# GuoleiSun/VSS-CFFM

Hardware: AMD Instinct MI355X
Metric: clips/sec (fwd+bwd) CFFM-B1 480x480 T=4 hot path (CFFA+CFM, decoder_focal depth 2) (higher is better)
Workload: dtype f32 in/out, f32 accumulate; MFMA operands: split-bf16 (hi+lo, ~2^-17) in the Linear GEMMs, f16 in QK^T/AV

## Files before the change

vss_cffm_amd/csrc/cffm_hip.hip:

```cpp
#include "cfm_attn_kernels.h"
#include "clip_kernels.h"
#include "rowops_kernels.h"
#include "gtc_kernels.h"
#include "gemm.h"
#include "segfuse_kernels.h"
#include "segloss_kernels.h"
#include "headfuse_kernels.h"
#include "kmeans_kernels.h"

#include <stdarg.h>
#include <stdio.h>

#include "../../include/cffm_hip.h"

static thread_local char g_err[512] = "";

static int fail(int code, const char* fmt, ...) {
    va_list ap;
    va_start(ap, fmt);
    vsnprintf(g_err, sizeof(g_err), fmt, ap);
    va_end(ap);
    return code;
}
#define CHECK_LAUNCH(name)                                                                        \
// ... 1061 lines not shown
    }
#endif
    CFFM_LAUNCH(k_gtc_attn_bwd, (nwg, CFFM_HEADS, B), (256), (size_t)gtb_lds(K), st, q_raw, q_b, kv_raw, kv_b, o, dout, lse, dq_raw, rec, T, K);
    CFFM_LAUNCH(k_gtc_dkv_sum, (K, CFFM_HEADS, B), (64), 0, st, (const float*)rec, nwg, K, dkv);
    CHECK_LAUNCH("gtc_attn_bwd");
    return 0;
}

#ifndef MLP_MT
#define MLP_MT 2
#endif
#define MLP_D 4
static int mlp_lds_grant() {
#ifndef CFFM_EMU
    static bool granted = false;
    if (!granted) {
        if (hipFuncSetAttribute((const void*)k_mlp_fwd<MLP_MT, MLP_D>, hipFuncAttributeMaxDynamicSharedMemorySize, PNL_FUSED_LDS(MLP_MT)) != hipSuccess ||
            hipFuncSetAttribute((const void*)k_mlp_bwd<MLP_MT, MLP_D>, hipFuncAttributeMaxDynamicSharedMemorySize, PNL_FUSED_LDS(MLP_MT)) != hipSuccess)
            return -1;
        granted = true;
    }
#endif
    return 0;
}
static int panel_mt(long M) {
    const long w2 = (M + 31) / 32, w3 = (M + 47) / 48;
    return ((w3 + 255) / 256) * 3 < ((w2 + 255) / 256) * 2 ? 3 : 2;
}
extern "C++" {
template <int MT, int NTW, bool A_PRE, int EPI>
static int panel_gemm_launch(const float* A, int lda, long M, int K, const float* wf, float* Cout, int ldc, const float* bias, void* aux,
                             hipStream_t st, float* colrec = nullptr, float* a_t = nullptr) {
    auto kern = k_panel_gemm<MT, NTW, 2, 4, A_PRE, EPI>;
#ifndef CFFM_EMU
    static bool granted = false;
    if (!granted) {
        if (hipFuncSetAttribute((const void*)kern, hipFuncAttributeMaxDynamicSharedMemorySize, PNL_LDS(MT)) != hipSuccess) return -1;
        granted = true;
    }
#endif
    CFFM_LAUNCH(kern, ((unsigned)((M + 16 * MT - 1) / (16 * MT))), (PNL_THREADS), PNL_LDS(MT), st, A, lda, (int)M, K, (const f32x4*)wf, Cout, ldc, bias, aux, colrec, (f32x4*)a_t);
    return 0;
}
}
static int panel_qkv_fwd(const float* x_s, const float* wf, const float* b, h16* qkv16, long M, hipStream_t st, float* x_t = nullptr) {
    return panel_mt(M) == 3 ? panel_gemm_launch<3, 6, true, 3>(x_s, 256, M, 256, wf, nullptr, 768, b, qkv16, st, nullptr, x_t)
                            : panel_gemm_launch<2, 6, true, 3>(x_s, 256, M, 256, wf, nullptr, 768, b, qkv16, st, nullptr, x_t);
}
static long panel_qkv_records(long M) { return (M + 16 * panel_mt(M) - 1) / (16 * panel_mt(M)); }
static int panel_qkv_dx(const float* dqkv, const float* wfn, float* dx, long M, hipStream_t st, float* colrec = nullptr, float* dqkv_t = nullptr) {
    return panel_mt(M) == 3 ? panel_gemm_launch<3, 2, false, 0>(dqkv, 768, M, 768, wfn, dx, 256, nullptr, nullptr, st, colrec, dqkv_t)
                            : panel_gemm_launch<2, 2, false, 0>(dqkv, 768, M, 768, wfn, dx, 256, nullptr, nullptr, st, colrec, dqkv_t);
}
#ifndef CFFM_DW_STREAM_DEFAULT
#define CFFM_DW_STREAM_DEFAULT 0
#endif
static int g_dw_stream = CFFM_DW_STREAM_DEFAULT;
static int dw_stream_sw() { return g_dw_stream; }
int cffm_dw_stream(int on) { const int was = g_dw_stream; if (on >= 0) g_dw_stream = on != 0; return was; }

static long cffm_mlp_records(long NP) { return (NP + 16 * MLP_MT - 1) / (16 * MLP_MT); }

int cffm_panel_pack_weight(const float* w, int N, int K, int form, float* w_frag, void* stream) {
    REQUIRE(w && w_frag && N >= 16 && K >= 16 && N % 32 == 0 && K % 32 == 0 && (form == 0 || form == 1), "panel_pack_weight: bad arguments");
    CFFM_LAUNCH(k_pnl_pack_weight, ((unsigned)(((long)N * K / 8 + 255) / 256)), (256), 0, (hipStream_t)stream, w, N, K, form, (f32x4*)w_frag);
    CHECK_LAUNCH("panel_pack_weight");
    return 0;
}

static int cffm_mlp_fwd_tfrag(const float* ao, const float* xt, long xt_bs, int rows_per_batch, const float* wp_f, const float* w1_f, const float* w2_f,
                              const float* bp, const float* b1, const float* b2, const float* g2, const float* be2, float* x1, float* z2s, float* mean2,
                              float* rstd2, float* hraw, float* acts, float* x2, float* ao_t, float* z2_t, float* act_t, long NP, void* stream) {
    REQUIRE(NP >= 0 && NP < (1L << 21) && rows_per_batch >= 1, "mlp_fwd: bad sizes");
    if (!NP) return 0;
    REQUIRE(ao && xt && wp_f && w1_f && w2_f && bp && b1 && b2 && g2 && be2 && x1 && mean2 && rstd2 && hraw && x2, "mlp_fwd: null");
    REQUIRE(!mlp_lds_grant(), "mlp_fwd: LDS grant failed");
    PROF2(ST_MLP_FWD);
    MlpFwdArgs a;
    a.ao = ao; a.xt = xt; a.xt_bs = xt_bs; a.rows_per_batch = rows_per_batch;
    a.wp = (const f32x4*)wp_f; a.w1 = (const f32x4*)w1_f; a.w2 = (const f32x4*)w2_f;
    a.bp = bp; a.b1 = b1; a.b2 = b2; a.g2 = g2; a.be2 = be2;
    a.x1 = x1; a.z2s = z2s; a.mean2 = mean2; a.rstd2 = rstd2; a.hraw = hraw; a.acts = acts; a.x2 = x2; a.NP = (int)NP;
    a.ao_t = (f32x4*)ao_t; a.z2_t = (f32x4*)z2_t; a.act_t = (f32x4*)act_t;
    CFFM_LAUNCH((k_mlp_fwd<MLP_MT, MLP_D>), ((unsigned)cffm_mlp_records(NP)), (PNL_THREADS), PNL_FUSED_LDS(MLP_MT), (hipStream_t)stream, a);
    CHECK_LAUNCH("mlp_fwd");
    return 0;
}
int cffm_mlp_fwd(const float* ao, const float* xt, long xt_bs, int rows_per_batch, const float* wp_f, const float* w1_f, const float* w2_f,
                 const float* bp, const float* b1, const float* b2, const float* g2, const float* be2, float* x1, float* z2s, float* mean2,
                 float* rstd2, float* hraw, float* acts, float* x2, long NP, void* stream) {
    REQUIRE(z2s || !NP, "mlp_fwd: null");
    return cffm_mlp_fwd_tfrag(ao, xt, xt_bs, rows_per_batch, wp_f, w1_f, w2_f, bp, b1, b2, g2, be2, x1, z2s, mean2, rstd2, hraw, acts, x2, nullptr, nullptr,
                              nullptr, NP, stream);
}

static int cffm_mlp_bwd_tfrag(const float* dout, const float* hraw, const float* b1, const float* x1, const float* mean2, const float* rstd2,
                              const float* g2, const float* w2_n, const float* w1_n, const float* wp_n, float* dhs, float* dx1, float* dao, float* dg2,
                              float* dbe2, float* db1, float* db2, float* dbp, float* dout_t, float* dh_t, float* dx1_t, long NP, void* stream) {
    REQUIRE(NP >= 0 && NP < (1L << 21), "mlp_bwd: bad sizes");
    if (!NP) return 0;
    REQUIRE(dout && hraw && b1 && x1 && mean2 && rstd2 && g2 && w2_n && w1_n && wp_n && dx1 && dao, "mlp_bwd: null");
    REQUIRE(!mlp_lds_grant(), "mlp_bwd: LDS grant failed");
    PROF2(ST_MLP_BWD);
    hipStream_t st = (hipStream_t)stream;
    const int nrec = (int)cffm_mlp_records(NP);
    float* rec = red_scratch((size_t)nrec * 2048, st);
// ... 327 lines not shown
        DwsPlan P4;
        if (stream_dw && dw_stream_plan(all4, 4, dw_stream_target(), &P4)) need = P4.part_floats;
        REQUIRE(!need || lib_scratch2(need), "block_backward: scratch allocation failed");
    }
    auto dw_group = [&](const cffm_wgrad* wg, const GemmTNPre* pre, int n, hipStream_t s, int target, void (*after)(hipStream_t)) -> int {
        if (!stream_dw) return gemm_tn_group((const GemmTN*)wg, n, s, pre, s == st ? lib_scratch : lib_scratch2, target, after);
        DwsPlan P;
        if (!dw_stream_plan((const GemmTN*)wg, n, dw_stream_target(), &P)) return -1;
        float* part = P.part_floats ? (s == st ? lib_scratch : lib_scratch2)(P.part_floats) : nullptr;
        if (P.part_floats && !part) return -1;
        return dw_group_stream((const GemmTN*)wg, n, s, part, dw_stream_target(), after);
    };
    const cffm_wgrad wg_qkv = {stream_dw ? dqkv_t : dqkv, stream_dw ? ws + L.zall_t : ws + L.zall, gr->qkv_w, NR, 768, CFFM_C};
    const cffm_wgrad wg_fc1 = {dact, ws + L.z2, gr->fc1_w, NP, CFFM_HID, CFFM_C};
    const cffm_wgrad wg_fc2 = {stream_dw ? dout_t : dout, ws + L.act, gr->fc2_w, NP, CFFM_C, CFFM_HID};
    const cffm_wgrad wg_proj = {stream_dw ? dx1_t : dx1, stream_dw ? ws + L.ao_t : ws + L.ao, gr->proj_w, NP, CFFM_C, CFFM_C};
    {
        const float* wfn = ws + L.w_frag + PREP_WFLOATS;
        PROF(ST_GEMM);
        if (stream_dw)
            TRY(cffm_mlp_bwd_tfrag(dout, ws + L.hraw, p->fc1_b, ws + L.x1, ws + L.mean2, ws + L.rstd2, p->norm2_w, wfn + 768 * 256 + 256 * 256 + 1024 * 256,
                                   wfn + 768 * 256 + 256 * 256, wfn + 768 * 256, nullptr, dx1, dao, gr->norm2_w, gr->norm2_b, gr->fc1_b, gr->fc2_b, gr->proj_b,
                                   dout_t, dact, dx1_t, NP, stream));
        else
        TRY(cffm_mlp_bwd(dout, ws + L.hraw, p->fc1_b, ws + L.x1, ws + L.mean2, ws + L.rstd2, p->norm2_w, wfn + 768 * 256 + 256 * 256 + 1024 * 256,
                         wfn + 768 * 256 + 256 * 256, wfn + 768 * 256, dact, dx1, dao, gr->norm2_w, gr->norm2_b, gr->fc1_b, gr->fc2_b, gr->proj_b, NP,
                         stream));
        TRY(tail_flush(st));
        if (!one_group) {
            sa = side_fork(st, 0);
            void* stream_a = (void*)sa;
            const cffm_wgrad wga[2] = {wg_fc1, wg_fc2};
            const GemmTNPre prea[2] = {{1, 1, nullptr}, {0, 1, p->fc1_b}};
            {
                void* stream = stream_a;
                PROF2(ST_G_DW);
                REQUIRE(!dw_group(wga, prea, 2, sa, 320, nullptr), "block_backward: weight-gradient gemm failed");
            }
            side_mark(sa, st, 0);
        }
    }
    hipStream_t sb = st, s1 = st;
    float* dbp;
    int ng;
    {
        PROF(ST_ATTN_BWD);
#ifndef CFFM_EMU
        if (g_side.bias_pending[par]) {
            side_wait(st, g_side.bias_done[par]);
            g_side.bias_pending[par] = false;
        }
#endif
        TRY(attn_bwd_fused(g, ws + L.qkv, key_src, q_dst, (const h16*)(ws + L.bias), ws + L.ao, dao, ws + L.lse, dqkv, scratch + S.dkvp, &dbp, &ng, par, stream));
        TRY(attn_bwd_gather(g, inv_ptr, inv_idx, scratch + S.dkvp, dqkv, stream));
    }
    const long nrec = panel_qkv_records(NR);
    float* qkv_rec = red_scratch((size_t)nrec * 768, st);
    REQUIRE(qkv_rec, "block_backward: scratch allocation failed");
    {
        RedSegs segs;
        segs.nseg = 0;
        seg_add(segs, 0, 768, gr->qkv_b, 0);
        reduce_records(qkv_rec, (int)nrec, 768, 768, segs, st);
    }
    {
        if (!stream_dw) side_fork_mark(st, 2);
        PROF(ST_GEMM); PROF2(ST_G_QKV_DX);
        REQUIRE(!panel_qkv_dx(dqkv, ws + L.w_frag + PREP_WFLOATS, dzall, NR, st, qkv_rec, stream_dw ? dqkv_t : nullptr), "block_backward: q|k|v input-gradient gemm failed");
        if (stream_dw) side_fork_mark(st, 2);
    }
    auto side_b = [&]() -> int {
        sb = side_fork_take(st, 2);
        void* stream_b = (void*)sb;
        if (one_group) {
            const cffm_wgrad wg4[4] = {wg_qkv, wg_fc1, wg_fc2, wg_proj};
            const GemmTNPre pre4[4] = {{0, 1, nullptr}, {1, 1, nullptr}, {0, 1, p->fc1_b}, {0, 0, nullptr}};
            void* stream = stream_b;
            PROF(ST_GEMM); PROF2(ST_G_DW);
            REQUIRE(!dw_group(wg4, pre4, 4, sb, 480, dw_group_launched), "block_backward: weight-gradient gemm failed");
            sa = sb;
            side_mark(sa, st, 0);
            {
                PROF(ST_ATTN_BWD);
                s1 = sb;
                TRY(attn_bwd_bias_sum(dbp, ng, dbiasT, (void*)s1));
                TRY(cffm_bias_scatter(dbiasT, gr->rpb_own, gr->rpb_ring, gr->rpb_pool, (void*)s1));
            }
        } else {
            const cffm_wgrad wgb[2] = {wg_qkv, wg_proj};
            const GemmTNPre preb[2] = {{0, 1, nullptr}, {0, 0, nullptr}};
            {
                void* stream = stream_b;
                PROF(ST_GEMM); PROF2(ST_G_DW);
                REQUIRE(!dw_group(wgb, preb, 2, sb, 320, dw_group_launched), "block_backward: weight-gradient gemm failed");
            }
            PROF(ST_ATTN_BWD);
            s1 = sb;
            TRY(attn_bwd_bias_sum(dbp, ng, dbiasT, (void*)s1));
            TRY(cffm_bias_scatter(dbiasT, gr->rpb_own, gr->rpb_ring, gr->rpb_pool, (void*)s1));
        }
        return 0;
    };
    const bool side_late = stream_dw && one_group;
    if (!side_late) TRY(side_b());
    if (!side_late && (!one_group || dx_tgt == dout)) side_join(sa, st, 0);
#ifndef CFFM_EMU
    if (g_side.dw_pending[par ^ 1] && g_side.dw_dout[par ^ 1] == dx_tgt) {
        side_wait(st, g_side.dw_done[par ^ 1]);
        g_side.dw_pending[par ^ 1] = false;
    }
#endif
    TRY(ln_pool_bwd_tgt(g, x_tgt, tgt_bs, p->norm1_w, p->norm1_b, ws + L.M, ws + L.mean1, ws + L.rstd1, dzall, dx1, dx_tgt, dtgt_bs, cffa.rec,
                        stream));
    if (side_late) TRY(side_b());
#ifndef CFFM_EMU
    if (defer && sb != st && s1 != st && g_side.on) {
        if (g_tail.has) TRY(tail_flush(st));
        side_fork_mark(st, 3);
        if (s1 != sb) side_order(s1, sb);
        (void)hipEventRecord(g_side.tail_order, sb);
        g_tail.has = true; g_tail.jobs = g_rq.jobs; g_tail.parity = g_red_parity;
        g_rq.jobs.njob = 0; g_rq.active = false;
        g_side.dw_pending[par] = true;
        g_side.dw_dout[par] = dout;
        side_record(s1, st, g_side.bias_done[par]);
        g_side.bias_pending[par] = true;
        return 0;
    }
#endif
    hipStream_t s3 = side_fork(st, 3);
    if (sb != st && s3 != st) side_order(sb, s3);
    if (s1 != st && s3 != st && s1 != s3) side_order(s1, s3);
    reductions.finish_on(s3);
    CHECK_LAUNCH("block_backward reductions");
#ifndef CFFM_EMU
    if (defer && sb != st && s3 != st) {
        g_side.dw_pending[par] = true;
        g_side.dw_dout[par] = dout;
        side_record(s1, st, g_side.bias_done[par]);
        g_side.bias_pending[par] = s1 != st;
        side_record(s3, st, g_side.tail_done[g_red_parity]);
        g_side.tail_pending[g_red_parity] = true;
        return 0;
    }
#endif
    (void)defer;
    side_mark(s3, st, 1);
    side_join(s3, st, 1);
    if (sb != st && sb != s3) { side_mark(sb, st, 0); side_join(sb, st, 0); }
    return 0;
}

static int segf_maps(SegfMaps& mp, const int* h, const int* w, int nmaps, int H, int W, const char* who) {
    if (nmaps < 0 || nmaps > 3 || H < 1 || W < 1) return fail(-1, "%s: bad map count / size", who);
    mp.cnt = nmaps;
    mp.nseg = 0; mp.per_frame = 0;
// ... 797 lines not shown
```

vss_cffm_amd/csrc/cfm_attn_kernels.h:

```cpp
#pragma once
#include "cffa_kernels.h"

#define ATT_KS_STRIDE 32
#define ATT_SWZ(row) ((0x78 >> (((row) >> 1) & 6)) & 3)
#define ATT_ROW(row, chunk) ((row) * ATT_KS_STRIDE + 8 * ((chunk) ^ ATT_SWZ(row)))

__device__ __forceinline__ f32x4 vflag4(const float* vflag, int o) { return *(const f32x4*)(vflag + o); }
#define CFFM_FIRST_POOLED_KEY 181
#define ATT_FWD_LDS (2 * CFFM_NKEY_PAD * ATT_KS_STRIDE * sizeof(f16) + CFFM_NKEY_PAD * 4)
template <int NROWS = 0>
__device__ __forceinline__ f16x8 att_tr_frag(const f16* img, int r0, int c0, int lane) {
    const int i = lane & 15, row = r0 + 4 * (lane >> 4) + (i >> 2), col = c0 + 4 * (i & 3);
    int row2 = row + 16;
    if (NROWS > 0 && row2 >= NROWS) row2 -= 16;
    const f16x4 a = lds_tr4(img + ATT_ROW(row, col >> 3) + (col & 7));
    const f16x4 b = lds_tr4(img + ATT_ROW(row2, col >> 3) + (col & 7));
    return cat_f16x4(a, b);
}

__device__ __forceinline__ int att_tr_lane(int c0, int lane) {
    const int i = lane & 15, row = 4 * (lane >> 4) + (i >> 2), col = c0 + 4 * (i & 3);
    return ATT_ROW(row, col >> 3) + (col & 7);
}
__device__ __forceinline__ f16x8 att_tr_frag_at(const f16* img_r0, int lane_off, bool clamp_second = false) {
// ... 355 lines not shown
        if (wb == wb0 || ntile == 0) wait_vm0(); else if (ntile == 1) wait_vm<2>(); else wait_vm<4>();
        __syncthreads();
        const bool more = wb + 1 < wb1;
        if (more) dma_rows(n1, onx, bi ^ 1);
        const f16* Ks = img + bi * ATT_BK_IMG;
        const f16* Vs = Ks + CFFM_NKEY_PAD * ATT_KS_STRIDE;
        const f16* Q = Qs + bi * 64 * ATT_KS_STRIDE;
        const f16* dO = dOs + bi * 64 * ATT_KS_STRIDE;
        const float isc = sisc[bi];
#pragma unroll
        for (int u = 0; u < 2; ++u) {
            const int t = t0 + u;
            if (u < ntile) {
                sched_fence();
                const f16x8 kf = *(const f16x8*)(Ks + 512 * t + lrow);
                const f16x8 vf = *(const f16x8*)(Vs + 512 * t + lrow);
                const float mk = t >= 11 ? vfl[bi * CFFM_NKEY_PAD + 16 * t + l15] : 0.f;
                const f32x4 c0 = (f32x4){mk, mk, mk, mk};
                f16x4 ph[4], dsh[4];
#pragma unroll
                for (int qt = 0; qt < 4; ++qt) {
                    if (u == 0 && more) dma_piece(n1.b, onx, bi ^ 1, qt);
                    const f16x8 qf = *(const f16x8*)(Q + 512 * qt + lrow);
                    const f16x8 dof = *(const f16x8*)(dO + 512 * qt + lrow);
                    const f32x4 sv = mfma16x16x32_f16(qf, kf, mfma16x16x32_f16(bT[qt], u ? sel1 : sel0, c0));
                    const f32x4 dp = mfma16x16x32_f16(dof, vf, (f32x4){0.f, 0.f, 0.f, 0.f});
                    const f32x4 lq = *(const f32x4*)(lse2 + bi * 64 + 16 * qt + 4 * g), Dq = *(const f32x4*)(sD + bi * 64 + 16 * qt + 4 * g);
                    f32x4 pr, ds;
#pragma unroll
                    for (int r = 0; r < 4; ++r) {
                        pr[r] = fast_exp2(fmaf(sv[r], CFFM_LOG2E, -lq[r]));
                        ds[r] = pr[r] * (dp[r] - Dq[r]);
                    }
                    dB[u][qt] += ds * isc;
                    ph[qt] = to_f16x4(pr);
                    dsh[qt] = to_f16x4(ds);
                    *(f16x4*)(DS + (qt >> 1) * ATT_BK_DSROWS * ATT_KS_STRIDE + 512 * t + ((qt & 1) ? dsw1 : dsw0)) = dsh[qt];
                }
                if (u == 0 && more) {
                    dma_piece(n1.b, onx, bi ^ 1, 4);
                    if (wb + 3 < wb1) tab_issue(n3.w, r3);
                }
                f32x4 aK[2] = {(f32x4){0.f, 0.f, 0.f, 0.f}, (f32x4){0.f, 0.f, 0.f, 0.f}}, aV[2] = {aK[0], aK[0]};
#pragma unroll
                for (int a = 0; a < 2; ++a) {
                    const f16x8 pf = cat_f16x4(ph[2 * a], ph[2 * a + 1]), dsf = cat_f16x4(dsh[2 * a], dsh[2 * a + 1]);
#pragma unroll
                    for (int mt = 0; mt < 2; ++mt) {
                        aV[mt] = mfma16x16x32_f16(att_tr_frag_at(dO + 1024 * a, mt ? ltp1 : ltp0), pf, aV[mt]);
                        aK[mt] = mfma16x16x32_f16(att_tr_frag_at(Q + 1024 * a, mt ? ltp1 : ltp0), dsf, aK[mt]);
                    }
                }
                const uint32_t so = (uint32_t)(((long)wb * CFFM_NKEY_PAD + 16 * t) * 1024);
                const uint32_t vo = mk == 0.f ? (uint32_t)(l15 * 1024 + (h * 2 * CFFM_HD + 8 * g) * 2) : BUF_OOB;
                buf_st16_pair(rs_part, __builtin_bit_cast(f32x4, cat_f16x4(to_f16x4(aK[0]), to_f16x4(aK[1]))),
                              __builtin_bit_cast(f32x4, cat_f16x4(to_f16x4(aV[0]), to_f16x4(aV[1]))), vo, so, so + 64);
            }
        }
        if (more && ntile == 0) {
#pragma unroll
            for (int k = 0; k < 5; ++k) dma_piece(n1.b, onx, bi ^ 1, k);
            if (wb + 3 < wb1) tab_issue(n3.w, r3);
        }
        if (wb + 2 < wb1) {
            Ahead a;
            sched_fence();
            ahead_lds(r3 + 2 >= 3 ? r3 - 1 : r3 + 2, a);
            dma_prep(n2.w, a, onx);
        }
        if (more && wave < 9) {
            if (wave < 7) wait_vm<8>(); else if (wave == 7) wait_vm<6>(); else wait_vm<4>();
            if (wave < 8) rows_max();
        }
        __syncthreads();
        if (wave >= 8) {
            if (more) rows_convert(wb + 1, bi ^ 1);
        } else {
            const int qt = wave & 3, mt = wave >> 2;
            const f16* D = DS + (qt >> 1) * ATT_BK_DSROWS * ATT_KS_STRIDE;
            const int la = mt ? ltr1 : ltr0, lb = (qt & 1) ? ltr1 : ltr0;
            f32x4 dq = (f32x4){0.f, 0.f, 0.f, 0.f};
#pragma unroll
            for (int p = 0; p < 10; ++p)
                dq = mfma16x16x32_f16(att_tr_frag_at(Ks + 1024 * p, la, p == 9), att_tr_frag_at(D + 1024 * p, lb), dq);
            const int q = 16 * qt + l15;
            if (q < CFFM_WA)
                *(f32x4*)(dqkv + ((long)b * G.RC + w * CFFM_WA + q) * 768 + h * CFFM_HD + 16 * mt + 4 * g) = dq * (scale * isc);
        }
        cur = n1;
        r3 = r3 == 2 ? 0 : r3 + 1;
    }
    const buf_t rs_dbp = buf_make(dbias_part + (((long)grp * CFFM_HEADS + h) * CFFM_NKEY_PAD) * CFFM_NQ_PAD,
                                  (uint32_t)(CFFM_NKEY_PAD * CFFM_NQ_PAD * 4));
#pragma unroll
    for (int u = 0; u < 2; ++u)
#pragma unroll
        for (int qt = 0; qt < 4; qt += 2)
            if (u < ntile) {
                const uint32_t so = (uint32_t)(((16 * (t0 + u)) * CFFM_NQ_PAD + 16 * qt) * 4);
                buf_st16_pair(rs_dbp, dB[u][qt], dB[u][qt + 1], (uint32_t)((l15 * CFFM_NQ_PAD + 4 * g) * 4), so, so + 64);
            }
}

__global__ void __launch_bounds__(256) k_dkv_gather(Geo G, const int* __restrict__ inv_ptr, const int* __restrict__ inv_idx,
                                                     const float* __restrict__ dkv_part, float* __restrict__ dqkv) {
    const int lane = threadIdx.x & 63, row = blockIdx.x * 4 + (threadIdx.x >> 6), b = blockIdx.y;
    if (row >= G.RC) return;
    const int e0 = inv_ptr[row], e1 = inv_ptr[row + 1];
    const h16* part = (const h16*)dkv_part + (long)b * G.nW * CFFM_NKEY_PAD * 512 + 8 * lane;
    const float* scl = dkv_part + (long)G.B * G.nW * CFFM_NKEY_PAD * 256 + (long)b * G.nW * CFFM_HEADS + (lane >> 3);
    f32x4 a0 = (f32x4){0.f, 0.f, 0.f, 0.f}, a1 = a0;
    for (int eb = e0; eb < e1; eb += 64) {
        const int n = (e1 - eb < 64) ? e1 - eb : 64;
        const int mine = (lane < n) ? inv_idx[eb + lane] : 0;
        int e = 0;
        for (; e + 3 < n; e += 4) {
            const int i0 = __shfl(mine, e, 64), i1 = __shfl(mine, e + 1, 64), i2 = __shfl(mine, e + 2, 64), i3 = __shfl(mine, e + 3, 64);
            const h16x8 x0 = *(const h16x8*)(part + (long)i0 * 512), x1 = *(const h16x8*)(part + (long)i1 * 512);
            const h16x8 x2 = *(const h16x8*)(part + (long)i2 * 512), x3 = *(const h16x8*)(part + (long)i3 * 512);
            const float s0 = scl[(i0 / CFFM_NKEY_PAD) * CFFM_HEADS], s1 = scl[(i1 / CFFM_NKEY_PAD) * CFFM_HEADS];
            const float s2 = scl[(i2 / CFFM_NKEY_PAD) * CFFM_HEADS], s3 = scl[(i3 / CFFM_NKEY_PAD) * CFFM_HEADS];
#pragma unroll
            for (int c = 0; c < 4; ++c) {
                a0[c] += ((float)x0[c] * s0 + (float)x1[c] * s1) + ((float)x2[c] * s2 + (float)x3[c] * s3);
                a1[c] += ((float)x0[4 + c] * s0 + (float)x1[4 + c] * s1) + ((float)x2[4 + c] * s2 + (float)x3[4 + c] * s3);
            }
        }
        for (; e < n; ++e) {
            const int i0 = __shfl(mine, e, 64);
            const h16x8 x0 = *(const h16x8*)(part + (long)i0 * 512);
            const float s0 = scl[(i0 / CFFM_NKEY_PAD) * CFFM_HEADS];
#pragma unroll
            for (int c = 0; c < 4; ++c) { a0[c] += (float)x0[c] * s0; a1[c] += (float)x0[4 + c] * s0; }
        }
    }
    float* drow = dqkv + ((long)b * G.RC + row) * 768;
    const int dcol = 256 + 256 * ((lane >> 2) & 1) + CFFM_HD * (lane >> 3) + 8 * (lane & 3);
    *(f32x4*)(drow + dcol) = a0;
    *(f32x4*)(drow + dcol + 4) = a1;
    if (row >= CFFM_WA * G.nW) *(f32x4*)(drow + 4 * lane) = (f32x4){0.f, 0.f, 0.f, 0.f};
}
```

vss_cffm_amd/csrc/panel_kernels.h:

```cpp
#pragma once
#include "cffm_common.h"
#include "gemm_kernels.h"
#include "dws_kernels.h"

#define PNL_KC 256
#define PNL_THREADS 512
#define PNL_WAVES 8
__device__ __forceinline__ int pnl_off(int row, int chunk) { return row * PNL_KC + (((chunk ^ row) & 15) << 3) + ((chunk & 16) << 3); }
#define PNL_IMG(MT) (16 * (MT) * PNL_KC)
#define PNL_LDS(MT) (2 * 2 * PNL_IMG(MT) * 2 + 2 * PNL_THREADS * 16)

__device__ __host__ __forceinline__ long pnl_frag_unit(int jt, int ks, int h, int KS) { return ((long)(jt * KS + ks) * 2 + h) * 64; }

__device__ __forceinline__ void pnl_pack_weight(const float* __restrict__ W, int N, int K, bool nn, f32x4* __restrict__ dst, long item) {
    const int lane = (int)(item & 63);
    const long u = item >> 6;
    const int OUT = nn ? K : N, KS = (nn ? N : K) / 32;
    const int ks = (int)(u % KS), jt = (int)(u / KS);
    if (jt * 16 >= OUT) return;
    const int l15 = lane & 15, g = lane >> 4;
    bf16x8 hi, lo;
#pragma unroll
    for (int e = 0; e < 8; ++e) {
        const int o = 16 * jt + l15, c = 32 * ks + 8 * g + e;
        const float x = nn ? W[(long)c * K + o] : W[(long)o * K + c];
        hi[e] = (bf16)x;
        lo[e] = (bf16)(x - (float)hi[e]);
    }
    dst[pnl_frag_unit(jt, ks, 0, KS) + lane] = __builtin_bit_cast(f32x4, hi);
    dst[pnl_frag_unit(jt, ks, 1, KS) + lane] = __builtin_bit_cast(f32x4, lo);
}
__global__ void __launch_bounds__(256) k_pnl_pack_weight(const float* __restrict__ W, int N, int K, int nn, f32x4* __restrict__ dst) {
    const long item = (long)blockIdx.x * 256 + threadIdx.x;
    if (item < (long)N * K / 8) pnl_pack_weight(W, N, K, nn != 0, dst, item);
}

struct PnlPackJobs { const float* w[4]; f32x4* dst[4]; int N[4], K[4]; long end[4]; int n, nn; };
__global__ void __launch_bounds__(256) k_pnl_pack_weights(PnlPackJobs J) {
    long item = (long)blockIdx.x * 256 + threadIdx.x;
    int j = 0;
#pragma unroll
    for (int q = 0; q < 3; ++q)
        if (q + 1 < J.n && item >= J.end[q]) j = q + 1;
    if (j > 0) item -= J.end[j - 1];
    if (item < (long)J.N[j] * J.K[j] / 8) pnl_pack_weight(J.w[j], J.N[j], J.K[j], J.nn != 0, J.dst[j], item);
}

__device__ __forceinline__ void pnl_lds_barrier() {
#ifdef CFFM_EMU
    __syncthreads();
#else
    __builtin_amdgcn_fence(__ATOMIC_RELEASE, "workgroup", "local");
    __builtin_amdgcn_s_barrier();
    __builtin_amdgcn_fence(__ATOMIC_ACQUIRE, "workgroup", "local");
#endif
}

template <int MT>
struct PnlStage { f32x4 v[2 * MT]; };
template <int MT>
__device__ __forceinline__ void pnl_stage_load(PnlStage<MT>& r, buf_t rs, int lda, int m0, int kc0, int tid) {
#pragma unroll
    for (int it = 0; it < 2 * MT; ++it) {
// ... 158 lines not shown
    pnl_stage_store<MT, A_PRE>(sr, img, img + PNL_IMG(MT), tid);
    PNL_COLSUM_PUT(0)
    if (NCH > 1) pnl_stage_load<MT>(sr, rsa, lda, m0, PNL_KC, tid);
    pnl_lds_barrier();
    for (int c = 0; c < NCH; ++c) {
        PNL_COLSUM_GET(c)
        const bf16* hi = img + (c & 1) * 2 * PNL_IMG(MT);
        pnl_chunk_mma<MT, NTW, NT, D>(acc, ring, hi, hi + PNL_IMG(MT), st, jt0, 8 * c, l15, g, st, jt0, 8 * (c + 1));
        if (a_t) pnl_tfrag_store<MT>(hi, hi + PNL_IMG(MT), a_t, m0, 16 * c, K / 16, M, ((long)M + 31) / 32 * 32, wave, lane);
        if (c + 1 < NCH) {
            bf16* nx = img + ((c + 1) & 1) * 2 * PNL_IMG(MT);
            pnl_stage_store<MT, A_PRE>(sr, nx, nx + PNL_IMG(MT), tid);
            PNL_COLSUM_PUT(c + 1)
            if (c + 2 < NCH) pnl_stage_load<MT>(sr, rsa, lda, m0, (c + 2) * PNL_KC, tid);
            pnl_lds_barrier();
        }
    }
#undef PNL_COLSUM_PUT
#undef PNL_COLSUM_GET
    {
        static_assert(EPI == 0 || EPI == 3, "k_panel_gemm epilogue");
        constexpr int ESZ = (EPI == 3) ? 2 : 4, NCOL = PNL_WAVES * NTW * 16, ROWB = NCOL * ESZ + 32, UPR = NCOL * ESZ / 16;
        static_assert(16 * MT * ROWB <= PNL_LDS(MT), "panel output does not fit the image buffers");
        char* out = (char*)smem;
        __syncthreads();
#pragma unroll
        for (int t = 0; t < NTW; ++t) {
            const int n = 16 * (jt0 + t) + 4 * g;
            f32x4 bv = (f32x4){0.f, 0.f, 0.f, 0.f};
            if (bias) bv = *(const f32x4*)(bias + n);
#pragma unroll
            for (int i = 0; i < MT; ++i) {
                char* q = out + (16 * i + l15) * ROWB + n * ESZ;
                if (EPI == 3) {
                    const float sc = n < CFFM_C ? 0.17677669529663687f : 1.f;
                    typedef h16 h16x4 __attribute__((ext_vector_type(4)));
                    h16x4 o;
                    for (int e = 0; e < 4; ++e) o[e] = (h16)((acc[t][i][e] + bv[e]) * sc);
                    *(h16x4*)q = o;
                } else {
                    *(f32x4*)q = acc[t][i] + bv;
                }
            }
        }
        __syncthreads();
        char* dst = (EPI == 3) ? (char*)aux : (char*)C;
        for (int u = tid; u < 16 * MT * UPR; u += PNL_THREADS) {
            const int r = u / UPR, c = u % UPR;
            if (m0 + r < M) *(f32x4*)(dst + ((long)(m0 + r) * ldc) * ESZ + 16 * c) = *(const f32x4*)(out + r * ROWB + 16 * c);
        }
    }
}

__device__ __forceinline__ f32x4 pnl_pack_hl(bf16x4 h, bf16x4 l) {
    const f32x2_t a = __builtin_bit_cast(f32x2_t, h), b = __builtin_bit_cast(f32x2_t, l);
    return (f32x4){a[0], a[1], b[0], b[1]};
}
__device__ __forceinline__ void pnl_img_put(bf16* __restrict__ hi, bf16* __restrict__ lo, int row, int n, bf16x4 h, bf16x4 l) {
    const int o = pnl_off(row, n >> 3) + (n & 4);
    *(bf16x4*)(hi + o) = h;
    *(bf16x4*)(lo + o) = l;
}
__device__ __forceinline__ float pnl_sum_g(float v) {
    v += __shfl_xor(v, 16, 64);
    v += __shfl_xor(v, 32, 64);
    return v;
}
#define PNL_STORE4(p, v) (*(f32x4*)(p) = (v))
#define PNL_FUSED_LDS(MT) (6 * PNL_IMG(MT) * 2 + 2 * PNL_WAVES * 16 * (MT) * 4)

struct MlpFwdArgs {
    const float* ao;
    const float* xt; long xt_bs; int rows_per_batch;
    const f32x4 *wp, *w1, *w2;
    const float *bp, *b1, *b2, *g2, *be2;
    float *x1, *z2s , *mean2, *rstd2, *hraw, *acts , *x2;
    f32x4 *ao_t, *z2_t, *act_t;
    int NP;
};

template <int MT, int D, bool INFER = false>
__global__ void __launch_bounds__(PNL_THREADS) k_mlp_fwd(MlpFwdArgs a) {
    CFFM_DYN_SMEM(smem);
    bf16* P = (bf16*)smem;
    bf16* ACT = P + 2 * PNL_IMG(MT);
    float* red = (float*)(ACT + 4 * PNL_IMG(MT));
    const int tid = threadIdx.x, lane = tid & 63, wave = wave_uniform(tid >> 6), l15 = lane & 15, g = lane >> 4;
    const int m0 = blockIdx.x * 16 * MT, NP = a.NP;
    PnlStream sp, s1, s2;
    sp.rs = buf_make(a.wp, 256u * 256 * 4); sp.voff = lane * 16; sp.KS = 8;
    s1.rs = buf_make(a.w1, 1024u * 256 * 4); s1.voff = lane * 16; s1.KS = 8;
    s2.rs = buf_make(a.w2, 1024u * 256 * 4); s2.voff = lane * 16; s2.KS = 32;
    PnlRing<2, D> ring;
#pragma unroll
    for (int s = 0; s < D - 1; ++s) pnl_ring_load<2, D>(ring, s, sp, 2 * wave, s);
    uint32_t touch = 0;
    pnl_pin_vmem();
    {
        PnlStage<MT> sr;
        pnl_stage_load<MT>(sr, buf_make(a.ao, (uint32_t)((long)NP * 256 * 4)), 256, m0, 0, tid);
        pnl_pin_vmem();
        const uint32_t t0 = pnl_l2_touch(a.w1, 1024L * 256 * 4, tid), t1 = pnl_l2_touch(a.w2, 1024L * 256 * 4, tid);
        pnl_pin_vmem();
        pnl_stage_store<MT, false>(sr, P, P + PNL_IMG(MT), tid);
        touch = t0 ^ t1;
    }
// ... 327 lines not shown
```

vss_cffm_amd/geometry.py:

```python
import functools

import numpy as np

WS = 7
EXPAND = 3
NKEY = 289
NKEY_PAD = 304
POOLED_GROUPS = ((49, 1, 5, 2), (50, 1, 7, 3), (51, 2, 5, 2), (55, 3, 3, 1))


def padded(n):
    return (n + WS - 1) // WS * WS


@functools.lru_cache(maxsize=32)
def tables(h0, w0):
    hp, wp = padded(h0), padded(w0)
    gy, gx = hp // WS, wp // WS
    nw = gy * gx
    key_src = np.full((nw, NKEY_PAD), -1, dtype=np.int32)
    q_dst = np.full((nw, WS * WS), -1, dtype=np.int32)
    ii, jj = np.meshgrid(np.arange(WS), np.arange(WS), indexing='ij')
    ii, jj = ii.reshape(-1), jj.reshape(-1)
    keep = (((ii >= WS - EXPAND) | (jj >= WS - EXPAND), +EXPAND, +EXPAND),
            ((ii >= WS - EXPAND) | (jj < EXPAND), +EXPAND, -EXPAND),
            ((ii < EXPAND) | (jj >= WS - EXPAND), -EXPAND, +EXPAND),
            ((ii < EXPAND) | (jj < EXPAND), -EXPAND, -EXPAND))
    for wy in range(gy):
        for wx in range(gx):
            w = wy * gx + wx
            y, x = WS * wy + ii, WS * wx + jj
            q_dst[w] = np.where((y < h0) & (x < w0), y * w0 + x, -1)
            key_src[w, :49] = w * 49 + np.arange(49)
            n = 49
            for sel, oy, ox in keep:
                yy, xx = (y[sel] + oy) % hp, (x[sel] + ox) % wp
                key_src[w, n:n + yy.size] = ((yy // WS) * gx + xx // WS) * 49 + (yy % WS) * WS + xx % WS
                n += yy.size
            for off, s, kk, pad in POOLED_GROUPS:
                a, b = np.meshgrid(np.arange(kk), np.arange(kk), indexing='ij')
                u, v = s * wy - pad + a.reshape(-1), s * wx - pad + b.reshape(-1)
                ok = (u >= 0) & (u < gy * s) & (v >= 0) & (v < gx * s)
                key_src[w, n:n + kk * kk] = np.where(ok, off * nw + u * (gx * s) + v, -1)
                n += kk * kk
            assert n == NKEY
    key_src.setflags(write=False)
    q_dst.setflags(write=False)
    return key_src, q_dst


@functools.lru_cache(maxsize=32)
def inverse_tables(h0, w0):
    key_src, _ = tables(h0, w0)
    nw = key_src.shape[0]
    flat = key_src.reshape(-1)
    slots = np.nonzero(flat >= 0)[0].astype(np.int32)
    rows = flat[slots]
    order = np.argsort(rows, kind='stable')
    inv_idx = np.ascontiguousarray(slots[order])
    counts = np.bincount(rows, minlength=64 * nw)
    inv_ptr = np.zeros(64 * nw + 1, dtype=np.int32)
    inv_ptr[1:] = np.cumsum(counts)
    return inv_ptr, inv_idx
```

Baseline: 2931.

## Fuse dK/dV scatter-gather into the q|k|v input-gradient panel GEMM

When the separate weight-gradient stream is off, the dK/dV partial gather (inverse-index reduction) is folded into a new panel GEMM kernel. The kernel streams gathered rows into the LDS operand images chunk by chunk, overlapping the gathers with MFMA work on the previous chunk, and writes the reduced dqkv back with its column sums. The dK/dV partial layout is changed to a head-contiguous order to match, and rows are assigned to panels with a skewed interleave for load balance. This removes one full pass over dqkv and a kernel launch, but the fused kernel needs more LDS and registers and the side-stream join timing is also changed.

Result: slower. 2730 (-6.8%).

```diff
diff --git a/vss_cffm_amd/csrc/cffm_hip.hip b/vss_cffm_amd/csrc/cffm_hip.hip
--- a/vss_cffm_amd/csrc/cffm_hip.hip
+++ b/vss_cffm_amd/csrc/cffm_hip.hip
@@ -1137,6 +1137,27 @@
     return panel_mt(M) == 3 ? panel_gemm_launch<3, 2, false, 0>(dqkv, 768, M, 768, wfn, dx, 256, nullptr, nullptr, st, colrec, dqkv_t)
                             : panel_gemm_launch<2, 2, false, 0>(dqkv, 768, M, 768, wfn, dx, 256, nullptr, nullptr, st, colrec, dqkv_t);
 }
+#define QKV_DX_SLOTS 2
+extern "C++" {
+template <int MT>
+static int panel_qkv_dx_gather_launch(const QkvDxGatherArgs& a, hipStream_t st) {
+    auto kern = k_qkv_dx_gather<MT, 4, QKV_DX_SLOTS>;
+#ifndef CFFM_EMU
+    static bool granted = false;
+    if (!granted) {
+        if (hipFuncSetAttribute((const void*)kern, hipFuncAttributeMaxDynamicSharedMemorySize, PNL_GATHER_LDS(MT)) != hipSuccess) return -1;
+        granted = true;
+    }
+#endif
+    CFFM_LAUNCH(kern, ((unsigned)((a.M + 16 * MT - 1) / (16 * MT))), (PNL_THREADS), PNL_GATHER_LDS(MT), st, a);
+    return 0;
+}
+}
+static int panel_qkv_dx_gather(const cffm_geom* g, float* dqkv, const float* dkv_part, const int* inv_ptr, const int* inv_idx, const float* wfn,
+                               float* dx, long M, hipStream_t st, float* colrec) {
+    const QkvDxGatherArgs a = {dqkv, dkv_part, inv_ptr, inv_idx, (const f32x4*)wfn, dx, colrec, (int)M, g->RC, g->nW, g->B};
+    return panel_mt(M) == 3 ? panel_qkv_dx_gather_launch<3>(a, st) : panel_qkv_dx_gather_launch<2>(a, st);
+}
 #ifndef CFFM_DW_STREAM_DEFAULT
 #define CFFM_DW_STREAM_DEFAULT 0
 #endif
@@ -1570,7 +1591,7 @@
         }
 #endif
         TRY(attn_bwd_fused(g, ws + L.qkv, key_src, q_dst, (const h16*)(ws + L.bias), ws + L.ao, dao, ws + L.lse, dqkv, scratch + S.dkvp, &dbp, &ng, par, stream));
-        TRY(attn_bwd_gather(g, inv_ptr, inv_idx, scratch + S.dkvp, dqkv, stream));
+        if (stream_dw) TRY(attn_bwd_gather(g, inv_ptr, inv_idx, scratch + S.dkvp, dqkv, stream));
     }
     const long nrec = panel_qkv_records(NR);
     float* qkv_rec = red_scratch((size_t)nrec * 768, st);
@@ -1582,10 +1603,13 @@
         reduce_records(qkv_rec, (int)nrec, 768, 768, segs, st);
     }
     {
-        if (!stream_dw) side_fork_mark(st, 2);
         PROF(ST_GEMM); PROF2(ST_G_QKV_DX);
-        REQUIRE(!panel_qkv_dx(dqkv, ws + L.w_frag + PREP_WFLOATS, dzall, NR, st, qkv_rec, stream_dw ? dqkv_t : nullptr), "block_backward: q|k|v input-gradient gemm failed");
-        if (stream_dw) side_fork_mark(st, 2);
+        if (stream_dw)
+            REQUIRE(!panel_qkv_dx(dqkv, ws + L.w_frag + PREP_WFLOATS, dzall, NR, st, qkv_rec, dqkv_t), "block_backward: q|k|v input-gradient gemm failed");
+        else
+            REQUIRE(!panel_qkv_dx_gather(g, dqkv, scratch + S.dkvp, inv_ptr, inv_idx, ws + L.w_frag + PREP_WFLOATS, dzall, NR, st, qkv_rec),
+                    "block_backward: q|k|v input-gradient gemm failed");
+        side_fork_mark(st, 2);
     }
     auto side_b = [&]() -> int {
         sb = side_fork_take(st, 2);
@@ -1619,7 +1643,7 @@
         }
         return 0;
     };
-    const bool side_late = stream_dw && one_group;
+    const bool side_late = one_group && (stream_dw || dx_tgt != dout);
     if (!side_late) TRY(side_b());
     if (!side_late && (!one_group || dx_tgt == dout)) side_join(sa, st, 0);
 #ifndef CFFM_EMU
diff --git a/vss_cffm_amd/csrc/cfm_attn_kernels.h b/vss_cffm_amd/csrc/cfm_attn_kernels.h
--- a/vss_cffm_amd/csrc/cfm_attn_kernels.h
+++ b/vss_cffm_amd/csrc/cfm_attn_kernels.h
@@ -431,9 +431,9 @@
                     }
                 }
                 const uint32_t so = (uint32_t)(((long)wb * CFFM_NKEY_PAD + 16 * t) * 1024);
-                const uint32_t vo = mk == 0.f ? (uint32_t)(l15 * 1024 + (h * 2 * CFFM_HD + 8 * g) * 2) : BUF_OOB;
+                const uint32_t vo = mk == 0.f ? (uint32_t)(l15 * 1024 + (h * CFFM_HD + 8 * g) * 2) : BUF_OOB;
                 buf_st16_pair(rs_part, __builtin_bit_cast(f32x4, cat_f16x4(to_f16x4(aK[0]), to_f16x4(aK[1]))),
-                              __builtin_bit_cast(f32x4, cat_f16x4(to_f16x4(aV[0]), to_f16x4(aV[1]))), vo, so, so + 64);
+                              __builtin_bit_cast(f32x4, cat_f16x4(to_f16x4(aV[0]), to_f16x4(aV[1]))), vo, so, so + 512);
             }
         }
         if (more && ntile == 0) {
@@ -481,13 +481,18 @@
             }
 }
 
+__device__ __forceinline__ float dkv_add4(float a, float x0, float s0, float x1, float s1, float x2, float s2, float x3, float s3) {
+    return a + ((x0 * s0 + x1 * s1) + (x2 * s2 + x3 * s3));
+}
+__device__ __forceinline__ float dkv_add1(float a, float x0, float s0) { return a + x0 * s0; }
+
 __global__ void __launch_bounds__(256) k_dkv_gather(Geo G, const int* __restrict__ inv_ptr, const int* __restrict__ inv_idx,
                                                      const float* __restrict__ dkv_part, float* __restrict__ dqkv) {
     const int lane = threadIdx.x & 63, row = blockIdx.x * 4 + (threadIdx.x >> 6), b = blockIdx.y;
     if (row >= G.RC) return;
     const int e0 = inv_ptr[row], e1 = inv_ptr[row + 1];
     const h16* part = (const h16*)dkv_part + (long)b * G.nW * CFFM_NKEY_PAD * 512 + 8 * lane;
-    const float* scl = dkv_part + (long)G.B * G.nW * CFFM_NKEY_PAD * 256 + (long)b * G.nW * CFFM_HEADS + (lane >> 3);
+    const float* scl = dkv_part + (long)G.B * G.nW * CFFM_NKEY_PAD * 256 + (long)b * G.nW * CFFM_HEADS + ((lane >> 2) & 7);
     f32x4 a0 = (f32x4){0.f, 0.f, 0.f, 0.f}, a1 = a0;
     for (int eb = e0; eb < e1; eb += 64) {
         const int n = (e1 - eb < 64) ? e1 - eb : 64;
@@ -501,8 +506,8 @@
             const float s2 = scl[(i2 / CFFM_NKEY_PAD) * CFFM_HEADS], s3 = scl[(i3 / CFFM_NKEY_PAD) * CFFM_HEADS];
 #pragma unroll
             for (int c = 0; c < 4; ++c) {
-                a0[c] += ((float)x0[c] * s0 + (float)x1[c] * s1) + ((float)x2[c] * s2 + (float)x3[c] * s3);
-                a1[c] += ((float)x0[4 + c] * s0 + (float)x1[4 + c] * s1) + ((float)x2[4 + c] * s2 + (float)x3[4 + c] * s3);
+                a0[c] = dkv_add4(a0[c], (float)x0[c], s0, (float)x1[c], s1, (float)x2[c], s2, (float)x3[c], s3);
+                a1[c] = dkv_add4(a1[c], (float)x0[4 + c], s0, (float)x1[4 + c], s1, (float)x2[4 + c], s2, (float)x3[4 + c], s3);
             }
         }
         for (; e < n; ++e) {
@@ -510,12 +515,11 @@
             const h16x8 x0 = *(const h16x8*)(part + (long)i0 * 512);
             const float s0 = scl[(i0 / CFFM_NKEY_PAD) * CFFM_HEADS];
 #pragma unroll
-            for (int c = 0; c < 4; ++c) { a0[c] += (float)x0[c] * s0; a1[c] += (float)x0[4 + c] * s0; }
+            for (int c = 0; c < 4; ++c) { a0[c] = dkv_add1(a0[c], (float)x0[c], s0); a1[c] = dkv_add1(a1[c], (float)x0[4 + c], s0); }
         }
     }
     float* drow = dqkv + ((long)b * G.RC + row) * 768;
-    const int dcol = 256 + 256 * ((lane >> 2) & 1) + CFFM_HD * (lane >> 3) + 8 * (lane & 3);
-    *(f32x4*)(drow + dcol) = a0;
-    *(f32x4*)(drow + dcol + 4) = a1;
+    *(f32x4*)(drow + 256 + 8 * lane) = a0;
+    *(f32x4*)(drow + 256 + 8 * lane + 4) = a1;
     if (row >= CFFM_WA * G.nW) *(f32x4*)(drow + 4 * lane) = (f32x4){0.f, 0.f, 0.f, 0.f};
 }
diff --git a/vss_cffm_amd/csrc/panel_kernels.h b/vss_cffm_amd/csrc/panel_kernels.h
--- a/vss_cffm_amd/csrc/panel_kernels.h
+++ b/vss_cffm_amd/csrc/panel_kernels.h
@@ -2,6 +2,7 @@
 #include "cffm_common.h"
 #include "gemm_kernels.h"
 #include "dws_kernels.h"
+#include "cfm_attn_kernels.h"
 
 #define PNL_KC 256
 #define PNL_THREADS 512
@@ -9,6 +10,7 @@
 __device__ __forceinline__ int pnl_off(int row, int chunk) { return row * PNL_KC + (((chunk ^ row) & 15) << 3) + ((chunk & 16) << 3); }
 #define PNL_IMG(MT) (16 * (MT) * PNL_KC)
 #define PNL_LDS(MT) (2 * 2 * PNL_IMG(MT) * 2 + 2 * PNL_THREADS * 16)
+#define PNL_GATHER_LDS(MT) (PNL_LDS(MT) + PNL_WAVES * 2 * (MT) * 64 * 4)
 
 __device__ __host__ __forceinline__ long pnl_frag_unit(int jt, int ks, int h, int KS) { return ((long)(jt * KS + ks) * 2 + h) * 64; }
 
@@ -273,6 +275,225 @@
     }
 }
 
+struct QkvDxGatherArgs {
+    float* dqkv;
+    const float* dkv_part;
+    const int *inv_ptr, *inv_idx;
+    const f32x4* Wf;
+    float* C;
+    float* colrec;
+    int M, RC, nW, B;
+};
+#define QKV_DX_SKEW 13
+__device__ __host__ __forceinline__ int qkv_dx_row(int p, int r, int P) { return P * r + (p + QKV_DX_SKEW * r) % P; }
+__device__ __forceinline__ int wave_readlane(int v, int l) {
+#ifdef CFFM_EMU
+    return __shfl(v, l, 64);
+#else
+    return __builtin_amdgcn_readlane(v, l);
+#endif
+}
+template <int MT, int D, int NSLOT>
+__global__ void __launch_bounds__(PNL_THREADS) k_qkv_dx_gather(QkvDxGatherArgs a) {
+    CFFM_DYN_SMEM(smem);
+    bf16* img = (bf16*)smem;
+    f32x4* csum = (f32x4*)(img + 4 * PNL_IMG(MT));
+    constexpr int NIT = 2 * MT, K = 768, KS = K / 32;
+    int* lists = (int*)(csum + 2 * PNL_THREADS);
+    static_assert(8 % NSLOT == 0 && NSLOT >= 1, "a chunk's eight steps go round the slots");
+    typedef h16 h16x4 __attribute__((ext_vector_type(4)));
+    const int tid = threadIdx.x, lane = tid & 63, wave = wave_uniform(tid >> 6), l15 = lane & 15, g = lane >> 4;
+    const int P = gridDim.x, p = blockIdx.x, M = a.M, fine = CFFM_WA * a.nW;
+    const buf_t rsq = buf_make(a.dqkv, (uint32_t)((long)M * 768 * 4));
+    const buf_t rsp = buf_make(a.dkv_part, (uint32_t)((long)a.B * a.nW * CFFM_NKEY_PAD * 512 * 2));
+    const buf_t rss = buf_make(a.dkv_part + (long)a.B * a.nW * CFFM_NKEY_PAD * 256, (uint32_t)((long)a.B * a.nW * CFFM_HEADS * 4));
+    PnlStream st;
+    st.rs = buf_make(a.Wf, 256u * K * 4);
+    st.voff = lane * 16;
+    st.KS = KS;
+    const int jt0 = wave * 2;
+    const f32x4 z4 = (f32x4){0.f, 0.f, 0.f, 0.f};
+    f32x4 acc[2][MT];
+#pragma unroll
+    for (int t = 0; t < 2; ++t)
+#pragma unroll
+        for (int i = 0; i < MT; ++i) acc[t][i] = z4;
+    PnlRing<2, D> ring;
+#pragma unroll
+    for (int s = 0; s < D - 1; ++s) pnl_ring_load<2, D>(ring, s, st, jt0, s);
+    pnl_pin_vmem();
+    int pm = 0, pe0 = 0, pe1 = 0, pinfo = 0;
+    if (lane < NIT) {
+        const int m = qkv_dx_row(p, wave + 8 * lane, P);
+        pm = m;
+        if (m < M) {
+            const int b = m / a.RC, row = m - b * a.RC;
+            pe0 = a.inv_ptr[row];
+            pe1 = a.inv_ptr[row + 1];
+            pinfo = 1 | (row >= fine ? 2 : 0) | (b << 2);
+        }
+    }
+#ifndef CFFM_EMU
+    asm volatile("" : "+v"(pe0), "+v"(pe1));
+#endif
+    int* wlist = lists + wave * (NIT * 64);
+    auto list_fill = [&](int it, int from) {
+        const int e0 = wave_readlane(pe0, it) + from, e1 = wave_readlane(pe1, it);
+        wlist[it * 64 + lane] = lane < e1 - e0 ? a.inv_idx[e0 + lane] : 0;
+#ifdef CFFM_EMU
+        emu::wave_barrier();
+#endif
+    };
+#pragma unroll
+    for (int it = 0; it < NIT; ++it) list_fill(it, 0);
+    struct Tag { int n, last, it; };
+    Tag tag[NSLOT];
+    h16x4 gx[NSLOT][4];
+    float gs[NSLOT][4];
+#pragma unroll
+    for (int s = 0; s < NSLOT; ++s) tag[s] = Tag{0, 0, 0};
+    int gi_it = 0, gi_e = 0, gi_e1 = 0, gi_e0 = 0;
+    uint32_t gi_pb = 0, gi_sb = 0;
+    int chunk = 1, done = 0;
+    bf16* gimg = img;
+    f32x4 ga = z4, cs = z4;
+    auto row_begin = [&](int it) {
+        gi_it = it;
+        gi_e = gi_e0 = wave_readlane(pe0, it);
+        gi_e1 = wave_readlane(pe1, it);
+        if (gi_e1 - gi_e0 > 64) list_fill(it, 0);
+        const uint32_t b = (uint32_t)wave_readlane(pinfo, it) >> 2;
+        gi_pb = b * (uint32_t)a.nW * (CFFM_NKEY_PAD * 1024u);
+        gi_sb = b * (uint32_t)a.nW * (CFFM_HEADS * 4u);
+    };
+    auto issue = [&](int slot) {
+        Tag t = Tag{0, 0, 0};
+        if (gi_it < NIT) {
+            const int rem = gi_e1 - gi_e, pos = gi_e - gi_e0;
+            t.n = rem >= 4 ? 4 : rem;
+            if (pos >= 64 && (pos & 63) == 0) list_fill(gi_it, pos);
+            const int* lp = wlist + gi_it * 64 + (pos & 63);
+#pragma unroll
+            for (int k = 0; k < 4; ++k)
+                if (k < t.n) {
+                    const uint32_t i = (uint32_t)wave_uniform(lp[k]);
+                    gx[slot][k] = __builtin_bit_cast(h16x4, buf_ld8(rsp, (uint32_t)((chunk - 1) * 512 + lane * 8), gi_pb + i * 1024u));
+                    gs[slot][k] = buf_ld4(rss, (uint32_t)((lane >> 3) * 4), gi_sb + (i / CFFM_NKEY_PAD) * (CFFM_HEADS * 4u));
+                }
+            gi_e += t.n;
+            t.it = gi_it;
+            t.last = gi_e == gi_e1;
+            if (t.last) {
+                if (gi_it + 1 < NIT) row_begin(gi_it + 1);
+                else gi_it = NIT;
+            }
+        }
+        tag[slot] = t;
+    };
+    auto consume = [&](int slot) {
+        const Tag t = tag[slot];
+        if (t.n == 4) {
+#pragma unroll
+            for (int c = 0; c < 4; ++c)
+                ga[c] = dkv_add4(ga[c], (float)gx[slot][0][c], gs[slot][0], (float)gx[slot][1][c], gs[slot][1], (float)gx[slot][2][c], gs[slot][2],
+                                 (float)gx[slot][3][c], gs[slot][3]);
+        } else {
+#pragma unroll
+            for (int k = 0; k < 3; ++k)
+                if (k < t.n) {
+#pragma unroll
+                    for (int c = 0; c < 4; ++c) ga[c] = dkv_add1(ga[c], (float)gx[slot][k][c], gs[slot][k]);
+                }
+        }
+        if (t.last) {
+            bf16x4 h, l;
+            split4(ga, h, l);
+            const int o = pnl_off(wave + 8 * t.it, lane >> 1) + 4 * (lane & 1);
+            *(bf16x4*)(gimg + o) = h;
+            *(bf16x4*)(gimg + PNL_IMG(MT) + o) = l;
+            const int m = wave_readlane(pm, t.it);
+            if (m < M) {
+                *(f32x4*)(a.dqkv + (long)m * 768 + chunk * PNL_KC + 4 * lane) = ga;
+                cs += ga;
+            }
+            ga = z4;
+            ++done;
+        }
+        tag[slot] = Tag{0, 0, 0};
+    };
+    auto gstep = [&](int s) {
+        const int slot = (s + NSLOT - 1) % NSLOT;
+        consume(slot);
+        issue(slot);
+    };
+    auto gather_begin = [&](int c) {
+        chunk = c;
+        gimg = img + (c & 1) * 2 * PNL_IMG(MT);
+        done = 0;
+        cs = z4;
+        row_begin(0);
+#pragma unroll
+        for (int s = 0; s < NSLOT - 1; ++s) issue(s);
+    };
+    PnlStage<MT> sr;
+#pragma unroll
+    for (int it = 0; it < NIT; ++it) {
+        const int m = wave_readlane(pm, it), info = wave_readlane(pinfo, it);
+        sr.v[it] = z4;
+        if (info & 2) *(f32x4*)(a.dqkv + (long)m * 768 + 4 * lane) = z4;
+        else if (info & 1) sr.v[it] = buf_ld16(rsq, (uint32_t)(lane * 16), (uint32_t)m * (768u * 4));
+    }
+    pnl_stage_store<MT, false>(sr, img, img + PNL_IMG(MT), tid);
+    if (a.colrec) {
+        f32x4 s_ = sr.v[0];
+#pragma unroll
+        for (int it = 1; it < NIT; ++it) s_ += sr.v[it];
+        csum[tid] = s_;
+    }
+    pnl_lds_barrier();
+    gather_begin(1);
+    auto colsum_get = [&](int c) {
+        if (a.colrec && wave == c) {
+            const f32x4* p_ = csum + (c & 1) * PNL_THREADS + lane;
+            f32x4 t_ = p_[0];
+#pragma unroll
+            for (int w = 1; w < PNL_WAVES; ++w) t_ += p_[64 * w];
+            *(f32x4*)(a.colrec + (long)p * K + c * PNL_KC + 4 * lane) = t_;
+        }
+    };
+    for (int c = 0; c < 2; ++c) {
+        colsum_get(c);
+        const bf16* hi = img + (c & 1) * 2 * PNL_IMG(MT);
+        pnl_chunk_mma<MT, 2, 2, D>(acc, ring, hi, hi + PNL_IMG(MT), st, jt0, 8 * c, l15, g, st, jt0, 8 * (c + 1), gstep);
+        while (done < NIT) {
+#pragma unroll
+            for (int q = 0; q < NSLOT; ++q) gstep(q);
+        }
+        if (a.colrec) csum[((c + 1) & 1) * PNL_THREADS + tid] = cs;
+        pnl_lds_barrier();
+        if (c == 0) gather_begin(2);
+    }
+    colsum_get(2);
+    pnl_chunk_mma<MT, 2, 2, D>(acc, ring, img, img + PNL_IMG(MT), st, jt0, 16, l15, g, st, jt0, 24);
+    {
+        constexpr int ROWB = 256 * 4 + 32, UPR = 256 * 4 / 16;
+        static_assert(16 * MT * ROWB <= PNL_LDS(MT), "panel output does not fit the image buffers");
+        char* out = (char*)smem;
+        __syncthreads();
+#pragma unroll
+        for (int t = 0; t < 2; ++t)
+#pragma unroll
+            for (int i = 0; i < MT; ++i) *(f32x4*)(out + (16 * i + l15) * ROWB + (16 * (jt0 + t) + 4 * g) * 4) = acc[t][i];
+        __syncthreads();
+        static_assert(UPR == 64, "a wave stores the rows it staged");
+#pragma unroll
+        for (int it = 0; it < NIT; ++it) {
+            const int m = wave_readlane(pm, it);
+            if (m < M) *(f32x4*)((char*)a.C + (long)m * 1024 + 16 * lane) = *(const f32x4*)(out + (wave + 8 * it) * ROWB + 16 * lane);
+        }
+    }
+}
+
 __device__ __forceinline__ f32x4 pnl_pack_hl(bf16x4 h, bf16x4 l) {
     const f32x2_t a = __builtin_bit_cast(f32x2_t, h), b = __builtin_bit_cast(f32x2_t, l);
     return (f32x4){a[0], a[1], b[0], b[1]};
diff --git a/vss_cffm_amd/geometry.py b/vss_cffm_amd/geometry.py
--- a/vss_cffm_amd/geometry.py
+++ b/vss_cffm_amd/geometry.py
@@ -62,3 +62,15 @@
     inv_ptr = np.zeros(64 * nw + 1, dtype=np.int32)
     inv_ptr[1:] = np.cumsum(counts)
     return inv_ptr, inv_idx
+
+
+def qkv_dx_panels(m):
+    w2, w3 = -(-m // 32), -(-m // 48)
+    rows = 48 if -(-w3 // 256) * 3 < -(-w2 // 256) * 2 else 32
+    return -(-m // rows), rows
+
+
+def qkv_dx_panel_rows(m, skew=13):
+    P, R = qkv_dx_panels(m)
+    p, r = np.arange(P)[:, None], np.arange(R)[None, :]
+    return P * r + (p + skew * r) % P
```
